# TaiseiNiman/SimpleGaussianSplat_tk71

Measured on AMD Instinct MI355X. Metric: splat-pixel pairs blended per second (grouped cumprod fwd+bwd), higher is better.
Workload: dtype f32; 1 GPU; cfg3: 1920x1080, 1000000 Gaussians, mean 80 splats/pixel (deep heavy-tailed lists); pairs_per_gpu=166335639, pixel_groups_per_gpu=2073600, bytes_per_pair=32, tiles_left_to_the_follow_up_kernel=0, world_size_checked=1, tiles_resolved_through_the_descriptor_tree=1258

## Files before the change

include/grouped_cumprod_hip.h:

```cpp
#ifndef GROUPED_CUMPROD_HIP_H
#define GROUPED_CUMPROD_HIP_H

#include <stddef.h>
#include <stdint.h>

#ifdef __cplusplus
extern "C" {
#endif

#define GCP_OK 0
#define GCP_ERR_INVALID_ARGUMENT 1
#define GCP_ERR_WORKSPACE 2
#define GCP_ERR_HIP 3

#define GCP_ABI_VERSION 4

int gcp_abi_version(void);

const char* gcp_source_hash(void);

int gcp_last_hip_error(void);

const char* gcp_status_string(int status);

size_t gcp_workspace_bytes(int64_t n);

int gcp_workspace_init(void* ws, size_t ws_bytes, void* stream);

int gcp_cumprod_forward(const float* x, const int32_t* key, float* y, int64_t n,
                        void* ws, size_t ws_bytes, void* stream);

int gcp_cumsum_forward(const float* x, const int32_t* key, float* y, int64_t n,
                       void* ws, size_t ws_bytes, void* stream);

int gcp_cumprod_backward(const float* param, const float* param_cumprod,
                         const float* grad_out, const int32_t* inv, float* grad_in,
                         const int32_t* inv_len, int64_t n, int64_t n_groups,
                         void* ws, size_t ws_bytes, void* stream);

int gcp_cumsum_reverse(const float* x, const int32_t* key, float* y, int64_t n,
                       void* ws, size_t ws_bytes, void* stream);

int gcp_cumprod_forward_indexed(const float* x, const int32_t* sorted_key, const int32_t* index, float* y, int64_t n,
                                void* ws, size_t ws_bytes, void* stream);
int gcp_cumsum_forward_indexed(const float* x, const int32_t* sorted_key, const int32_t* index, float* y, int64_t n,
                               void* ws, size_t ws_bytes, void* stream);
int gcp_cumsum_reverse_indexed(const float* x, const int32_t* sorted_key, const int32_t* index, float* y, int64_t n,
                               void* ws, size_t ws_bytes, void* stream);

int gcp_cumprod_forward_carry(const float* x, const int32_t* inv, const float* carry, float* y,
                              int64_t n, int64_t n_groups, void* ws, size_t ws_bytes, void* stream);
int gcp_cumsum_forward_carry(const float* x, const int32_t* inv, const float* carry, float* y,
                             int64_t n, int64_t n_groups, void* ws, size_t ws_bytes, void* stream);
int gcp_cumsum_reverse_carry(const float* x, const int32_t* inv, const float* carry, float* y,
                             int64_t n, int64_t n_groups, void* ws, size_t ws_bytes, void* stream);

int gcp_check_groups(const int32_t* inv, const int32_t* inv_len, int64_t n,
                     int64_t n_groups, int64_t* n_bad, void* stream);

int gcp_check_permutation(const int32_t* index, int64_t n, int64_t* n_bad, void* stream);
int gcp_check_group_ids(const int32_t* inv, int64_t n, int64_t n_groups, int64_t* n_bad, void* stream);
int gcp_set_validate_operands(int on);

int gcp_tile_elems(void);
int gcp_last_fallback_tiles(void* ws, void* stream, int64_t* n_tiles);
int gcp_set_lookback_wait_us(int64_t us);
int gcp_last_lookback_tiles(void* ws, void* stream, int64_t* n_tiles);



int gcp_tile_grid(int32_t width, int32_t height, int32_t* tiles_x, int32_t* tiles_y);

size_t gcp_scan_i32_workspace_bytes(int64_t n);
int gcp_exclusive_scan_i32(const int32_t* in, int32_t* out, int64_t n, void* ws, size_t ws_bytes,
                           void* stream);

int gcp_bin_tiles_count(const int32_t* start_xy, const int32_t* end_xy, int64_t n_gauss,
                        int32_t width, int32_t height, int32_t* tile_off,
                        int64_t* n_tile_pairs_host, void* ws, size_t ws_bytes, void* stream);
size_t gcp_bin_workspace_bytes(int64_t n_gauss, int64_t n_tile_pairs);
int gcp_bin_tiles_fill(const int32_t* start_xy, const int32_t* end_xy, int64_t n_gauss,
                       int32_t width, int32_t height, const int32_t* tile_off,
                       int64_t n_tile_pairs, int32_t* tile_start, int32_t* tile_list, void* ws,
                       size_t ws_bytes, void* stream);

int gcp_bin_tiles(const int32_t* start_xy, const int32_t* end_xy, int64_t n_gauss, int32_t width,
                  int32_t height, int64_t capacity, int32_t* tile_off, int32_t* tile_start,
                  int32_t* tile_list, int32_t* info, void* ws, size_t ws_bytes, void* stream);

size_t gcp_blend_checkpoint_floats(int64_t n_tile_pairs, int32_t width, int32_t height);
int gcp_blend_forward(const int32_t* start_xy, const int32_t* end_xy, const float* mean_xy,
                      const float* vinv, const float* opacity, const float* l_d, int64_t n_gauss,
                      int32_t width, int32_t height, const int32_t* tile_start,
                      const int32_t* tile_list, float* image, float* t_ckpt, void* stream);

size_t gcp_blend_backward_workspace_bytes(int64_t n_tile_pairs);
int gcp_blend_backward(const int32_t* start_xy, const int32_t* end_xy, const float* mean_xy,
                       const float* vinv, const float* opacity, const float* l_d, int64_t n_gauss,
                       int32_t width, int32_t height, const int32_t* tile_off,
                       int64_t n_tile_pairs, const int32_t* tile_start, const int32_t* tile_list,
                       const float* t_ckpt, const float* grad_image, float* grad_mean,
                       float* grad_vinv, float* grad_opacity, float* grad_l, void* ws,
                       size_t ws_bytes, void* stream);

int gcp_blend_forward_depth(const int32_t* start_xy, const int32_t* end_xy, const float* mean_xy,
                            const float* vinv, const float* opacity, const float* l_d, const float* depth,
                            const float* background, int64_t n_gauss, int32_t width, int32_t height,
                            const int32_t* tile_start, const int32_t* tile_list, float* image,
                            float* depth_map, float* alpha_map, float* t_ckpt, void* stream);
size_t gcp_blend_backward_depth_workspace_bytes(int64_t n_tile_pairs, int32_t width, int32_t height);
int gcp_blend_backward_depth(const int32_t* start_xy, const int32_t* end_xy, const float* mean_xy,
                             const float* vinv, const float* opacity, const float* l_d, const float* depth,
                             const float* background, int64_t n_gauss, int32_t width, int32_t height,
                             const int32_t* tile_off, int64_t n_tile_pairs, const int32_t* tile_start,
                             const int32_t* tile_list, const float* t_ckpt, const float* grad_image,
                             const float* grad_depth_map, const float* grad_alpha_map, float* grad_mean,
                             float* grad_vinv, float* grad_opacity, float* grad_l, float* grad_depth,
                             float* grad_background, void* ws, size_t ws_bytes, void* stream);

size_t gcp_sort_workspace_bytes(int64_t n);
int gcp_sort_pairs_u32(const uint32_t* keys_in, int64_t n, int32_t key_bits, uint32_t* keys_out,
// ... 274 lines not shown
```

simplegaussiansplat_tk71_amd/_lib.py:

```python
import ctypes
import os

from . import _build
from ._build import LIB_PATH

_c_void_p = ctypes.c_void_p
_i64 = ctypes.c_int64
_sz = ctypes.c_size_t
_i32 = ctypes.c_int32

SIGNATURES = {
    "gcp_abi_version": (ctypes.c_int, []),
    "gcp_source_hash": (ctypes.c_char_p, []),
    "gcp_last_hip_error": (ctypes.c_int, []),
    "gcp_status_string": (ctypes.c_char_p, [ctypes.c_int]),
    "gcp_workspace_bytes": (_sz, [_i64]),
    "gcp_workspace_init": (ctypes.c_int, [_c_void_p, _sz, _c_void_p]),
    "gcp_cumprod_forward": (ctypes.c_int, [_c_void_p, _c_void_p, _c_void_p, _i64, _c_void_p, _sz, _c_void_p]),
    "gcp_cumsum_forward": (ctypes.c_int, [_c_void_p, _c_void_p, _c_void_p, _i64, _c_void_p, _sz, _c_void_p]),
    "gcp_cumsum_reverse": (ctypes.c_int, [_c_void_p, _c_void_p, _c_void_p, _i64, _c_void_p, _sz, _c_void_p]),
    "gcp_cumprod_forward_indexed": (ctypes.c_int, [_c_void_p] * 4 + [_i64, _c_void_p, _sz, _c_void_p]),
    "gcp_cumsum_forward_indexed": (ctypes.c_int, [_c_void_p] * 4 + [_i64, _c_void_p, _sz, _c_void_p]),
    "gcp_cumsum_reverse_indexed": (ctypes.c_int, [_c_void_p] * 4 + [_i64, _c_void_p, _sz, _c_void_p]),
    "gcp_cumprod_forward_carry": (ctypes.c_int, [_c_void_p] * 4 + [_i64, _i64, _c_void_p, _sz, _c_void_p]),
    "gcp_cumsum_forward_carry": (ctypes.c_int, [_c_void_p] * 4 + [_i64, _i64, _c_void_p, _sz, _c_void_p]),
    "gcp_cumsum_reverse_carry": (ctypes.c_int, [_c_void_p] * 4 + [_i64, _i64, _c_void_p, _sz, _c_void_p]),
    "gcp_cumprod_backward": (
        ctypes.c_int,
        [_c_void_p, _c_void_p, _c_void_p, _c_void_p, _c_void_p, _c_void_p, _i64, _i64, _c_void_p, _sz, _c_void_p],
    ),
    "gcp_check_groups": (ctypes.c_int, [_c_void_p, _c_void_p, _i64, _i64, ctypes.POINTER(_i64), _c_void_p]),
    "gcp_check_permutation": (ctypes.c_int, [_c_void_p, _i64, ctypes.POINTER(_i64), _c_void_p]),
    "gcp_check_group_ids": (ctypes.c_int, [_c_void_p, _i64, _i64, ctypes.POINTER(_i64), _c_void_p]),
    "gcp_set_validate_operands": (ctypes.c_int, [ctypes.c_int]),
    "gcp_tile_elems": (ctypes.c_int, []),
    "gcp_last_fallback_tiles": (ctypes.c_int, [_c_void_p, _c_void_p, ctypes.POINTER(_i64)]),
    "gcp_last_lookback_tiles": (ctypes.c_int, [_c_void_p, _c_void_p, ctypes.POINTER(_i64)]),
    "gcp_set_lookback_wait_us": (ctypes.c_int, [_i64]),
    "gcp_tile_grid": (ctypes.c_int, [_i32, _i32, ctypes.POINTER(_i32), ctypes.POINTER(_i32)]),
    "gcp_scan_i32_workspace_bytes": (_sz, [_i64]),
    "gcp_exclusive_scan_i32": (ctypes.c_int, [_c_void_p, _c_void_p, _i64, _c_void_p, _sz, _c_void_p]),
    "gcp_bin_tiles_count": (
        ctypes.c_int,
        [_c_void_p, _c_void_p, _i64, _i32, _i32, _c_void_p, ctypes.POINTER(_i64), _c_void_p, _sz, _c_void_p],
    ),
    "gcp_bin_workspace_bytes": (_sz, [_i64, _i64]),
    "gcp_bin_tiles_fill": (
        ctypes.c_int,
        [_c_void_p, _c_void_p, _i64, _i32, _i32, _c_void_p, _i64, _c_void_p, _c_void_p, _c_void_p, _sz, _c_void_p],
    ),
    "gcp_bin_tiles": (
        ctypes.c_int,
        [_c_void_p, _c_void_p, _i64, _i32, _i32, _i64, _c_void_p, _c_void_p, _c_void_p, _c_void_p, _c_void_p, _sz, _c_void_p],
    ),
    "gcp_blend_checkpoint_floats": (_sz, [_i64, _i32, _i32]),
    "gcp_blend_forward": (
        ctypes.c_int,
        [_c_void_p] * 6 + [_i64, _i32, _i32, _c_void_p, _c_void_p, _c_void_p, _c_void_p, _c_void_p],
    ),
    "gcp_blend_backward_workspace_bytes": (_sz, [_i64]),
    "gcp_blend_backward": (
        ctypes.c_int,
        [_c_void_p] * 6 + [_i64, _i32, _i32, _c_void_p, _i64] + [_c_void_p] * 8 + [_c_void_p, _sz, _c_void_p],
    ),
    "gcp_blend_forward_depth": (ctypes.c_int, [_c_void_p] * 8 + [_i64, _i32, _i32] + [_c_void_p] * 7),
    "gcp_blend_backward_depth_workspace_bytes": (_sz, [_i64, _i32, _i32]),
    "gcp_blend_backward_depth": (ctypes.c_int, [_c_void_p] * 8 + [_i64, _i32, _i32, _c_void_p, _i64] + [_c_void_p] * 13 + [_sz, _c_void_p]),
    "gcp_gather_f32": (ctypes.c_int, [_c_void_p, _c_void_p, _c_void_p, _i64, _c_void_p]),
    "gcp_unsort_finish": (ctypes.c_int, [_c_void_p] * 5 + [_i64, _i32, _c_void_p]),
    "gcp_sort_workspace_bytes": (_sz, [_i64]),
    "gcp_sort_pairs_u32": (ctypes.c_int, [_c_void_p, _i64, _i32, _c_void_p, _c_void_p, _c_void_p, _sz, _c_void_p]),
    "gcp_sort_rects": (ctypes.c_int, [_c_void_p, _i64, _i32, _i32, _c_void_p, _c_void_p, _c_void_p, _sz, _c_void_p]),
    "gcp_rects_key_range": (ctypes.c_int, [_c_void_p, _i64, _c_void_p, _c_void_p]),
    "gcp_compact_workspace_bytes": (_sz, [_i64]),
    "gcp_compact_finish": (ctypes.c_int, [_c_void_p, _c_void_p, _i64, _i64, _i32, _c_void_p, _c_void_p, _c_void_p, _c_void_p, _c_void_p, _sz, _c_void_p]),
    "gcp_pairs_finish_prepare": (ctypes.c_int, [_c_void_p, _c_void_p, _i64, _c_void_p]),
    "gcp_pairs_finish_boxes": (ctypes.c_int, [_c_void_p, _c_void_p, _i64, _i32, _i32] + [_c_void_p] * 6 + [_i64, _i32, _c_void_p, _i32, _c_void_p]),
    "gcp_compact_kept_workspace_bytes": (_sz, [_i64]),
    "gcp_compact_kept_count": (ctypes.c_int, [_c_void_p, _c_void_p, _i64, _i64, _i64, _c_void_p, _c_void_p, _sz, _c_void_p]),
    "gcp_compact_kept_write": (ctypes.c_int, [_c_void_p, _c_void_p, _i64, _i64, _c_void_p, _c_void_p, _sz, _c_void_p]),
    "gcp_rects_cut_workspace_bytes": (_sz, [_i64, _i64, _i64, _i32, _i64]),
    "gcp_rects_cut": (ctypes.c_int, [_c_void_p, _i32, _i64, _i64, _i64, _i32, _i64] + [_c_void_p] * 6 + [_sz, _c_void_p]),
    "gcp_pixels_range": (ctypes.c_int, [_c_void_p, _i32, _i64, _c_void_p, _c_void_p]),
    "gcp_pixels_min_workspace_bytes": (_sz, [_i32, _i32]),
    "gcp_pixels_min": (ctypes.c_int, [_c_void_p, _i32, _c_void_p, _i64, _i32, _i32, _c_void_p, _c_void_p, _i64, _c_void_p, _c_void_p, _sz, _c_void_p]),
    "gcp_rects_rows_workspace_bytes": (_sz, [_i64]),
    "gcp_rects_rows_capacity": (_i64, [_i64]),
    "gcp_rects_rows": (ctypes.c_int, [_c_void_p, _i64, _i64, _c_void_p, _c_void_p, _c_void_p, _c_void_p, _sz, _c_void_p]),
    "gcp_rects_rows_i64": (ctypes.c_int, [_c_void_p, _i64, _i64, _c_void_p, _c_void_p, _c_void_p, _c_void_p, _sz, _c_void_p]),
    "gcp_rows_rectangles_workspace_bytes": (_sz, [_i64]),
    "gcp_rows_rectangles": (ctypes.c_int, [_c_void_p, _c_void_p, _i64, _c_void_p, _c_void_p, _c_void_p, _sz, _c_void_p]),
    "gcp_rectangle_boxes": (ctypes.c_int, [_c_void_p, _c_void_p, _c_void_p, _i64, _i64, _c_void_p, _c_void_p, _c_void_p, _c_void_p]),
    "gcp_pairs_scan_boxes": (ctypes.c_int, [_c_void_p, _c_void_p, _i64, _i32, _i32] + [_c_void_p] * 5 + [_i64, _i32, _c_void_p, _c_void_p]),
    "gcp_box_sizes": (ctypes.c_int, [_c_void_p, _c_void_p, _i64, _i32, _i32, _c_void_p, _c_void_p]),
    "gcp_expand_rects": (ctypes.c_int, [_c_void_p, _c_void_p, _c_void_p, _i64, _i64, _i32, _i32, _c_void_p, _c_void_p, _c_void_p]),
    "gcp_pixel_lists_count": (ctypes.c_int, [_c_void_p, _c_void_p, _i64, _i32, _i32] + [_c_void_p] * 5),
    "gcp_pixel_lists_fill": (ctypes.c_int, [_c_void_p, _c_void_p, _i64, _i32, _i32] + [_c_void_p] * 8),
    "gcp_project_forward": (ctypes.c_int, [_c_void_p] * 7 + [_i64, _i32, _i32, _i32, _i32, ctypes.c_float] + [_c_void_p] * 5),
    "gcp_project_gather": (ctypes.c_int, [_c_void_p, _c_void_p, _i64] + [_c_void_p] * 11),
    "gcp_adam_step": (ctypes.c_int, [_c_void_p] * 4 + [_i64] + [ctypes.c_double] * 4 + [_i64, _c_void_p]),
    "gcp_adam_step_multi": (ctypes.c_int, [_i32] + [_c_void_p] * 10 + [ctypes.c_double] * 3 + [_c_void_p]),
    "gcp_ssim_blocks": (_i64, [_i64, _i32, _i32]),
    "gcp_ssim_l1_forward": (ctypes.c_int, [_c_void_p, _c_void_p, _i64, _i32, _i32, _c_void_p, ctypes.c_float, ctypes.c_float]
                            + [_c_void_p] * 5),
    "gcp_ssim_l1_backward": (ctypes.c_int, [_c_void_p] * 5 + [_i64, _i32, _i32, _c_void_p, _c_void_p, _c_void_p, _c_void_p]),
    "gcp_image_metrics": (ctypes.c_int, [_c_void_p, _c_void_p, _i64, _i32, _i32, _i32, _c_void_p, ctypes.c_float, ctypes.c_float, _i32]
                          + [_c_void_p] * 3),
    "gcp_exposure_blocks": (_i64, [_i64, _i32, _i32]),
    "gcp_ssim_l1_forward_exposure": (ctypes.c_int, [_c_void_p] * 3 + [_i64, _i32, _i32, _c_void_p, ctypes.c_float, ctypes.c_float]
                                     + [_c_void_p] * 5),
# ... 99 lines not shown
```

simplegaussiansplat_tk71_amd/csrc/gcp_scan.hip:

```cpp

#include <hip/hip_runtime.h>
#include <stdint.h>
#include <stdlib.h>
#include <atomic>
#include <mutex>

#include "gcp_device.hpp"
#include "grouped_cumprod_hip.h"

namespace gcp {
thread_local int t_last_hip_error = 0;
int hip_fail(hipError_t e) {
  t_last_hip_error = (int)e;
  return GCP_ERR_HIP;
}
}

namespace {
using namespace gcp;

typedef float float4_t __attribute__((ext_vector_type(4)));
typedef int int4_t __attribute__((ext_vector_type(4)));

enum : int { M_CUMPROD_FWD = 0, M_CUMSUM_FWD = 1, M_CUMPROD_BWD = 2, M_CUMSUM_REV = 3 };

constexpr int kThreads = 256;
constexpr int kWaves = 4;
constexpr int kRows = 4;
constexpr int kTile = 1024 * kRows;
constexpr int kLbBatch = 5;
constexpr int kLbBatchBwd = 3;
constexpr int kLbChunks = ((kTile / 256 - 1) / kLbBatch) * kLbBatch + 1;
constexpr int kFixBlocks = 256;
constexpr int kFixBlocksQuiet = 32;
constexpr int kWsHeaderBytes = 256;
constexpr int kHdrEpoch = 0;
constexpr int kHdrDone = 1;
constexpr int kHdrUnresolved = 2;
constexpr int kHdrTiles = 3;
constexpr int kHdrDescResolved = 5;
constexpr int kHdrAnyUnresolved = 6;
constexpr int kHdrBarrier = 7;
constexpr unsigned kDOpen = 1u;
constexpr unsigned kDUnresolved = 2u;
constexpr unsigned kDValid = 1u << 15;
constexpr unsigned kDTree = 1u << 16;
constexpr int kLevels = 4;
constexpr int kXcdChunk = 32;
constexpr int kXcdChunkIndexed = 128;
constexpr int kDescWaitUs = 200;

static_assert(kLbChunks * 256 == kTile, "the raw look-back window is exactly the previous tile (the descriptor walk starts at the tile before it)");
static_assert((kLbChunks - 1) % kLbBatch == 0, "chunks after the first are fetched kLbBatch at a time");
static_assert((kLbChunks - 1) % kLbBatchBwd == 0, "chunks after the first are fetched kLbBatchBwd at a time in the backward");

template <int MODE>
struct Mode {
  static constexpr bool kMul = (MODE == M_CUMPROD_FWD);
  static constexpr bool kRev = (MODE == M_CUMPROD_BWD || MODE == M_CUMSUM_REV);
  static constexpr bool kBwd = (MODE == M_CUMPROD_BWD);
  static constexpr int kBatch = kBwd ? kLbBatchBwd : kLbBatch;
};

template <bool MUL>
struct Monoid {
  static __device__ __forceinline__ float identity() { return MUL ? 1.0f : 0.0f; }
  static __device__ __forceinline__ float op(float a, float b) { return MUL ? a * b : a + b; }
};

struct ScanArgs {
  const float* in0;
  const float* in1;
  const float* in2;
  const int* key;
  const int* ends;
  i64 n_groups;
  const float* carry;
  const int* index;
  float* out;
  i64 n;
  i64 ntiles;
  unsigned long long* desc_sets;
  i64 lvl_off[kLevels + 1];
  unsigned* hdr;
  int xcd_remap;
  long long patience;
};

template <bool MUL>
__device__ __forceinline__ float wave_seg_scan(float v, int h, int lane) {
  typedef Monoid<MUL> M;
  const float id = M::identity();
  float t;
  t = dpp_f<0x111, 0xf>(id, v); v = M::op(v, (lane - 1 >= h) ? t : id);
  t = dpp_f<0x112, 0xf>(id, v); v = M::op(v, (lane - 2 >= h) ? t : id);
  t = dpp_f<0x114, 0xf>(id, v); v = M::op(v, (lane - 4 >= h) ? t : id);
  t = dpp_f<0x118, 0xf>(id, v); v = M::op(v, (lane - 8 >= h) ? t : id);
  t = dpp_f<0x142, 0xa>(id, v); v = M::op(v, ((lane & 48) - 1 >= h) ? t : id);
  t = dpp_f<0x143, 0xc>(id, v); v = M::op(v, (31 >= h) ? t : id);
  return v;
}

template <bool MUL>
__device__ __forceinline__ float wave_reduce(float v) {
  typedef Monoid<MUL> M;
  const float id = M::identity();
  v = M::op(v, dpp_f<0x111, 0xf>(id, v));
  v = M::op(v, dpp_f<0x112, 0xf>(id, v));
  v = M::op(v, dpp_f<0x114, 0xf>(id, v));
  v = M::op(v, dpp_f<0x118, 0xf>(id, v));
  v = M::op(v, dpp_f<0x142, 0xa>(id, v));
  v = M::op(v, dpp_f<0x143, 0xc>(id, v));
  return readlane_f(v, 63);
}

template <bool ALIGNED, bool NT = false>
__device__ __forceinline__ float4_t ld4(const float* p) {
  if (ALIGNED) {
    if (NT) return __builtin_nontemporal_load(reinterpret_cast<const float4_t*>(p));
    return *reinterpret_cast<const float4_t*>(p);
  }
  float4_t v; v.x = p[0]; v.y = p[1]; v.z = p[2]; v.w = p[3];
  return v;
}
template <bool ALIGNED, bool NT = false>
__device__ __forceinline__ int4_t ld4(const int* p) {
  if (ALIGNED) {
    if (NT) return __builtin_nontemporal_load(reinterpret_cast<const int4_t*>(p));
    return *reinterpret_cast<const int4_t*>(p);
  }
  int4_t v; v.x = p[0]; v.y = p[1]; v.z = p[2]; v.w = p[3];
  return v;
}
template <bool ALIGNED>
__device__ __forceinline__ void st4(float* p, float4_t v) {
  if (ALIGNED) {
    __builtin_nontemporal_store(v, reinterpret_cast<float4_t*>(p));
    return;
  }
  p[0] = v.x; p[1] = v.y; p[2] = v.z; p[3] = v.w;
}
__device__ __forceinline__ float4_t ld4_guard(const float* base, i64 p0, i64 n, float fill) {
  float4_t v;
  v.x = (p0 + 0 < n) ? base[p0 + 0] : fill;
  v.y = (p0 + 1 < n) ? base[p0 + 1] : fill;
  v.z = (p0 + 2 < n) ? base[p0 + 2] : fill;
  v.w = (p0 + 3 < n) ? base[p0 + 3] : fill;
  return v;
}
__device__ __forceinline__ int4_t ld4_guard(const int* base, i64 p0, i64 n, int fill) {
  int4_t v;
  v.x = (p0 + 0 < n) ? base[p0 + 0] : fill;
  v.y = (p0 + 1 < n) ? base[p0 + 1] : fill;
  v.z = (p0 + 2 < n) ? base[p0 + 2] : fill;
  v.w = (p0 + 3 < n) ? base[p0 + 3] : fill;
  return v;
}
template <bool ALIGNED, bool NT>
__device__ __forceinline__ float4_t ld4_indexed(const float* src, const int* index, i64 p, int4_t& idx) {
  idx = ld4<ALIGNED, NT>(index + p);
  float4_t v; v.x = src[idx.x]; v.y = src[idx.y]; v.z = src[idx.z]; v.w = src[idx.w];
  return v;
}
__device__ __forceinline__ float4_t ld4_indexed_guard(const float* src, const int* index, i64 p0, i64 n, float fill, int4_t& idx) {
  idx = ld4_guard(index, p0, n, 0);
  float4_t v;
  v.x = (p0 + 0 < n) ? src[idx.x] : fill;
  v.y = (p0 + 1 < n) ? src[idx.y] : fill;
  v.z = (p0 + 2 < n) ? src[idx.z] : fill;
  v.w = (p0 + 3 < n) ? src[idx.w] : fill;
  return v;
}
template <bool REV> __device__ __forceinline__ float4_t to_scan_order(float4_t v) {
  if (!REV) return v;
  float4_t r; r.x = v.w; r.y = v.z; r.z = v.y; r.w = v.x;
  return r;
}
template <bool REV> __device__ __forceinline__ int4_t to_scan_order(int4_t v) {
  if (!REV) return v;
  int4_t r; r.x = v.w; r.y = v.z; r.z = v.y; r.w = v.x;
  return r;
}

__device__ __forceinline__ i64 logical_tile(i64 b, i64 ntiles, int xcd_remap) {
  if (!xcd_remap) return b;
  const int lg = xcd_remap - 1 + 3;
  const i64 full = (ntiles >> lg) << lg;
  if (b >= full) return b;
  const i64 g = b >> lg, r = b & (((i64)1 << lg) - 1);
  return (g << lg) + ((r & 7) << (lg - 3)) + (r >> 3);
}

__device__ __forceinline__ unsigned long long pack_desc(float agg, unsigned flags, int first_head) {
  return ((unsigned long long)(flags | kDValid | ((unsigned)first_head << 2)) << 32) | __builtin_bit_cast(unsigned, agg);
}

constexpr int kEndIters = 4;
constexpr int kBitWords = 256 * kRows / 32;

__device__ __forceinline__ void wave_sync_lds() {
  __builtin_amdgcn_fence(__ATOMIC_RELEASE, "wavefront");
  __builtin_amdgcn_wave_barrier();
  __builtin_amdgcn_fence(__ATOMIC_ACQUIRE, "wavefront");
}

__device__ __forceinline__ bool group_ends(const ScanArgs& a, unsigned* bits, i64 wlo, i64 whi, int ga, int gb, int lane,
                                          i64& gend) {
  if (lane < kBitWords) bits[lane] = 0u;
  wave_sync_lds();
  if (!(wlo <= whi && ga >= 0 && ga <= gb && (i64)gb < a.n_groups && (i64)gb - ga + 2 <= 64 * kEndIters)) return false;
  const int last = gb - ga + 1;
  int e[kEndIters];
#pragma unroll
  for (int it = 0; it < kEndIters; ++it) {
    const int j = it * 64 + lane;
    e[it] = 0;
    if (j <= last && ga - 1 + j >= 0) e[it] = a.ends[ga - 1 + j];
  }
  bool bad = false;
  gend = 0;
#pragma unroll
  for (int it = 0; it < kEndIters; ++it) {
    const int j = it * 64 + lane;
    const int prev = dpp_i<0x138, 0xf>(it ? __builtin_amdgcn_readlane(e[it > 0 ? it - 1 : 0], 63) : 0, e[it]);
    const i64 ej = e[it];
    if (j >= 1 && j <= last) {
      bad = bad || e[it] <= prev;
      const i64 p = ej - 1;
      if (p >= wlo && p <= whi) atomicOr(bits + ((p - wlo) >> 5), 1u << ((p - wlo) & 31));
    }
    if (j == 0) bad = bad || ej > wlo;
    if (j == 1) bad = bad || ej <= wlo;
    if (j == last - 1) bad = bad || ej > whi;
    if (j == last) bad = bad || ej <= whi;
    if ((last >> 6) == it) gend = (i64)__builtin_amdgcn_readlane(e[it], last & 63);
  }
  wave_sync_lds();
  return __ballot(bad) == 0ull;
}

template <int MODE, bool ALIGNED, bool FULL, bool CARRY, bool FIXUP = false, bool INDEXED = false, bool INPLACE = false>
__device__ __forceinline__ void scan_tile(const ScanArgs& a, const i64 lt, float* s_wv, int* s_wf,
                                          float* s_tc, int* s_fh, unsigned* s_bits, const float fix_carry = 0.0f) {
  typedef Mode<MODE> MD;
  constexpr bool REV = MD::kRev;
  constexpr bool BWD = MD::kBwd;
  typedef Monoid<MD::kMul> M;
  const float id = M::identity();
  constexpr int WT = 256 * kRows;

  const int lane = threadIdx.x & 63;
  const int w = threadIdx.x >> 6;
  const i64 n = a.n;
  const i64 pt = REV ? (a.ntiles - 1 - lt) : lt;
  const i64 base = pt * (i64)kTile;
  unsigned long long* const desc = a.desc_sets + (a.hdr[kHdrEpoch] & 1u);

  const int wu = __builtin_amdgcn_readfirstlane(w);
  i64 wlo = 0, whi = -1;
  int ga = 0, gb = -1;
  if constexpr (BWD) {
    wlo = base + kTile - (i64)(wu + 1) * WT;
    whi = base + kTile - 1 - (i64)wu * WT;
    if (whi > n - 1) whi = n - 1;
  }

  const bool nt_main = w < kWaves - 1;
  float4_t v[kRows];
  int4_t kk[kRows];
  float4_t xp[BWD ? kRows : 1];
  int4_t ix[INDEXED ? kRows : 1];
  static_assert(!(INDEXED && BWD), "the backward has no indexed form");
  int4_t lb_ix;
  i64 p0[kRows];
  auto load_keys = [&](int r) {
    if (FULL) {
      if (nt_main) kk[r] = ld4<ALIGNED, true>(a.key + p0[r]);
      else kk[r] = ld4<ALIGNED>(a.key + p0[r]);
    } else {
      kk[r] = ld4_guard(a.key, p0[r], n, 0);
    }
    kk[r] = to_scan_order<REV>(kk[r]);
  };
#pragma unroll
  for (int r = 0; r < kRows; ++r) {
    const int q = w * WT + r * 256 + lane * 4;
    p0[r] = REV ? (base + kTile - 4 - q) : (base + q);
    if constexpr (!BWD) load_keys(r);
    if (FULL) {
      if (nt_main) {
        if constexpr (BWD) {
          v[r] = ld4<ALIGNED, true>(a.in2 + p0[r]) * ld4<ALIGNED, true>(a.in1 + p0[r]);
        } else if constexpr (INDEXED) {
          v[r] = ld4_indexed<ALIGNED, true>(a.in0, a.index, p0[r], ix[r]);
        } else {
          v[r] = ld4<ALIGNED, true>(a.in0 + p0[r]);
        }
      } else {
        if constexpr (BWD) {
          v[r] = ld4<ALIGNED>(a.in2 + p0[r]) * ld4<ALIGNED>(a.in1 + p0[r]);
        } else if constexpr (INDEXED) {
          v[r] = ld4_indexed<ALIGNED, false>(a.in0, a.index, p0[r], ix[r]);
        } else {
          v[r] = ld4<ALIGNED>(a.in0 + p0[r]);
        }
      }
      if constexpr (BWD) xp[r] = ld4<ALIGNED, true>(a.in0 + p0[r]);
    } else {
      if constexpr (BWD) {
        const float4_t g = ld4_guard(a.in2, p0[r], n, 0.0f);
        const float4_t c = ld4_guard(a.in1, p0[r], n, 0.0f);
        xp[r] = ld4_guard(a.in0, p0[r], n, 1.0f);
        v[r] = g * c;
      } else if constexpr (INDEXED) {
        v[r] = ld4_indexed_guard(a.in0, a.index, p0[r], n, id, ix[r]);
      } else {
        v[r] = ld4_guard(a.in0, p0[r], n, id);
      }
    }
    v[r] = to_scan_order<REV>(v[r]);
    if constexpr (BWD) xp[r] = to_scan_order<REV>(xp[r]);
  }

  if constexpr (BWD) {
    if (wlo <= whi) { ga = a.key[wlo]; gb = a.key[whi]; }
  }

  const i64 pn = REV ? (base + kTile - (i64)w * WT) : (base + (i64)w * WT - 1);
  const bool nb_exists = (pn >= 0) && (pn < n);
  int nbk = 0;
  if (!BWD && nb_exists) nbk = a.key[pn];

  const bool do_lb = !FIXUP && !INPLACE && (w == 0) && (lt > 0);
  float4_t lbv = {id, id, id, id};
  float4_t lbc = {id, id, id, id};
  int4_t lbk = {0, 0, 0, 0};
  i64 lbp = 0;
  if (do_lb) {
    lbp = REV ? (base + kTile + lane * 4) : (base - (lane * 4 + 4));
    if (!REV) {
      lbk = ld4<ALIGNED>(a.key + lbp);
      if constexpr (BWD) lbv = ld4<ALIGNED>(a.in2 + lbp) * ld4<ALIGNED>(a.in1 + lbp);
      else if constexpr (INDEXED) lbv = ld4_indexed<ALIGNED, false>(a.in0, a.index, lbp, lb_ix);
      else lbv = ld4<ALIGNED>(a.in0 + lbp);
    } else if (BWD && base + kTile + 256 <= n) {
      lbv = ld4<ALIGNED>(a.in2 + lbp);
      lbc = ld4<ALIGNED>(a.in1 + lbp);
    } else {
      if constexpr (!BWD) lbk = ld4_guard(a.key, lbp, n, 0);
      if constexpr (BWD) { lbv = ld4_guard(a.in2, lbp, n, 0.0f); lbc = ld4_guard(a.in1, lbp, n, 0.0f); }
      else if constexpr (INDEXED) lbv = ld4_indexed_guard(a.in0, a.index, lbp, n, id, lb_ix);
      else lbv = ld4_guard(a.in0, lbp, n, id);
    }
  }

  bool from_ends = false;
  i64 gend = 0;
  unsigned* const wbits = s_bits + kBitWords * wu;
  if constexpr (BWD) {
    from_ends = group_ends(a, wbits, wlo, whi, ga, gb, lane, gend);
    if (!from_ends) {
#pragma unroll
      for (int r = 0; r < kRows; ++r) load_keys(r);
      if (nb_exists) nbk = a.key[pn];
      if (do_lb) lbk = ld4_guard(a.key, lbp, n, 0);
    }
  }

  float s[kRows][4];
  float eloc[kRows];
  float rowtot[kRows];
  unsigned long long hmask[kRows];
  unsigned openbits = 0;
  unsigned lanes_open = 0;

#pragma unroll
  for (int r = 0; r < kRows; ++r) {
    int lane0_prev;
    if (r == 0) lane0_prev = nbk;
    else lane0_prev = __builtin_amdgcn_readlane(kk[r - 1].w, 63);
    const int pk = dpp_i<0x138, 0xf>(lane0_prev, kk[r].w);

    bool f0, f1, f2, f3;
    if (BWD && from_ends) {
      const int off = WT - 4 - r * 256 - lane * 4;
      const unsigned nib = (wbits[off >> 5] >> (off & 31)) & 0xfu;
      f0 = (nib >> 3) & 1u; f1 = (nib >> 2) & 1u; f2 = (nib >> 1) & 1u; f3 = nib & 1u;
      if (FULL) {
        f0 = f0 || ((lt == 0) && (w == 0) && (r == 0) && (lane == 0));
      } else {
        const i64 p = p0[r];
        f0 = (p + 3 < n) && (f0 || p + 3 == n - 1);
        f1 = (p + 2 < n) && (f1 || p + 2 == n - 1);
        f2 = (p + 1 < n) && (f2 || p + 1 == n - 1);
        f3 = (p + 0 < n) && (f3 || p + 0 == n - 1);
      }
    } else if (FULL) {
      const bool first_of_array = (lt == 0) && (w == 0) && (r == 0) && (lane == 0);
      f0 = first_of_array || (kk[r].x != pk);
      f1 = kk[r].y != kk[r].x;
      f2 = kk[r].z != kk[r].y;
      f3 = kk[r].w != kk[r].z;
    } else {
      bool val[4], pex[4];
#pragma unroll
      for (int k = 0; k < 4; ++k) {
        const i64 p = REV ? (p0[r] + 3 - k) : (p0[r] + k);
        val[k] = p < n;
        pex[k] = REV ? (p + 1 < n) : (p > 0);
      }
      f0 = val[0] && (!pex[0] || kk[r].x != pk);
      f1 = val[1] && (!pex[1] || kk[r].y != kk[r].x);
      f2 = val[2] && (!pex[2] || kk[r].z != kk[r].y);
      f3 = val[3] && (!pex[3] || kk[r].w != kk[r].z);
    }
    if constexpr (CARRY) {
      if (f0) v[r].x = M::op(a.carry[kk[r].x], v[r].x);
      if (f1) v[r].y = M::op(a.carry[kk[r].y], v[r].y);
      if (f2) v[r].z = M::op(a.carry[kk[r].z], v[r].z);
      if (f3) v[r].w = M::op(a.carry[kk[r].w], v[r].w);
    }
    const float s0 = v[r].x;
    const float s1 = f1 ? v[r].y : M::op(s0, v[r].y);
    const float s2 = f2 ? v[r].z : M::op(s1, v[r].z);
    const float s3 = f3 ? v[r].w : M::op(s2, v[r].w);
    s[r][0] = s0; s[r][1] = s1; s[r][2] = s2; s[r][3] = s3;
    const bool m0 = !f0, m1 = m0 && !f1, m2 = m1 && !f2, m3 = m2 && !f3;
    openbits |= ((unsigned)m0 | ((unsigned)m1 << 1) | ((unsigned)m2 << 2) | ((unsigned)m3 << 3)) << (4 * r);

    const unsigned long long mask = __ballot(!m3);
    hmask[r] = mask;
    const unsigned long long upto = mask & (~0ull >> (63 - lane));
    const int h = upto ? (63 - __clzll(upto)) : -1;
    if ((mask & ((1ull << lane) - 1ull)) == 0ull) lanes_open |= 1u << r;

    const float inc = wave_seg_scan<MD::kMul>(s3, h, lane);
    eloc[r] = dpp_f<0x138, 0xf>(id, inc);
    rowtot[r] = readlane_f(inc, 63);
  }

  float wagg = id;
  bool whead = false;
#pragma unroll
  for (int r = 0; r < kRows; ++r) {
    wagg = hmask[r] ? rowtot[r] : M::op(wagg, rowtot[r]);
    whead = whead || (hmask[r] != 0ull);
  }
  int wfh = WT;
#pragma unroll
  for (int r = kRows - 1; r >= 0; --r) {
    if (hmask[r]) {
      const int hl = __builtin_ctzll(hmask[r]);
      const unsigned ob = (unsigned)__builtin_amdgcn_readlane((int)openbits, hl);
      wfh = r * 256 + hl * 4 + __builtin_popcount((ob >> (4 * r)) & 0xfu);
    }
  }
  if (lane == 0) { s_wv[w] = wagg; s_wf[w] = whead ? 1 : 0; s_fh[w] = wfh; }

  if (w == 0) {
    float tc = FIXUP ? fix_carry : id;
    int unresolved = 0;
    if (do_lb) {
      const int k0 = from_ends ? 0 : __builtin_amdgcn_readfirstlane(kk[0].x);
      auto process = [&](float4_t cv, int4_t ck, i64 cp, int j) -> bool {
        const float4_t lv = REV ? cv : to_scan_order<true>(cv);
        const int4_t lk = REV ? ck : to_scan_order<true>(ck);
        bool c0, c1, c2, c3;
// ... 677 lines not shown
  GCP_HIP(hipMemsetAsync(ws, 0, ws_bytes, (hipStream_t)stream));
  return GCP_OK;
}

int gcp_cumprod_forward(const float* x, const int32_t* key, float* y, int64_t n, void* ws,
                        size_t ws_bytes, void* stream) {
  return launch_scan<M_CUMPROD_FWD>(x, nullptr, nullptr, key, y, n, ws, ws_bytes, stream);
}

int gcp_cumsum_forward(const float* x, const int32_t* key, float* y, int64_t n, void* ws,
                       size_t ws_bytes, void* stream) {
  return launch_scan<M_CUMSUM_FWD>(x, nullptr, nullptr, key, y, n, ws, ws_bytes, stream);
}

int gcp_cumsum_reverse(const float* x, const int32_t* key, float* y, int64_t n, void* ws,
                       size_t ws_bytes, void* stream) {
  return launch_scan<M_CUMSUM_REV>(x, nullptr, nullptr, key, y, n, ws, ws_bytes, stream);
}

int gcp_cumprod_forward_indexed(const float* x, const int32_t* sorted_key, const int32_t* index, float* y, int64_t n,
                                void* ws, size_t ws_bytes, void* stream) {
  if (n > 0 && !index) return GCP_ERR_INVALID_ARGUMENT;
  if (validate_operands()) {
    const int st = check_permutation_impl(index, n, nullptr, (hipStream_t)stream);
    if (st != GCP_OK) return st;
  }
  return launch_scan<M_CUMPROD_FWD>(x, nullptr, nullptr, sorted_key, y, n, ws, ws_bytes, stream, nullptr, index);
}

int gcp_cumsum_forward_indexed(const float* x, const int32_t* sorted_key, const int32_t* index, float* y, int64_t n,
                               void* ws, size_t ws_bytes, void* stream) {
  if (n > 0 && !index) return GCP_ERR_INVALID_ARGUMENT;
  if (validate_operands()) {
    const int st = check_permutation_impl(index, n, nullptr, (hipStream_t)stream);
    if (st != GCP_OK) return st;
  }
  return launch_scan<M_CUMSUM_FWD>(x, nullptr, nullptr, sorted_key, y, n, ws, ws_bytes, stream, nullptr, index);
}

int gcp_cumsum_reverse_indexed(const float* x, const int32_t* sorted_key, const int32_t* index, float* y, int64_t n,
                               void* ws, size_t ws_bytes, void* stream) {
  if (n > 0 && !index) return GCP_ERR_INVALID_ARGUMENT;
  if (validate_operands()) {
    const int st = check_permutation_impl(index, n, nullptr, (hipStream_t)stream);
    if (st != GCP_OK) return st;
  }
  return launch_scan<M_CUMSUM_REV>(x, nullptr, nullptr, sorted_key, y, n, ws, ws_bytes, stream, nullptr, index);
}

int gcp_cumprod_forward_carry(const float* x, const int32_t* inv, const float* carry, float* y, int64_t n,
                              int64_t n_groups, void* ws, size_t ws_bytes, void* stream) {
  if (n > 0 && (!carry || n_groups <= 0)) return GCP_ERR_INVALID_ARGUMENT;
  if (validate_operands()) {
    const int st = check_group_ids_impl(inv, n, n_groups, nullptr, (hipStream_t)stream);
    if (st != GCP_OK) return st;
  }
  return launch_scan<M_CUMPROD_FWD>(x, nullptr, nullptr, inv, y, n, ws, ws_bytes, stream, carry);
}

int gcp_cumsum_forward_carry(const float* x, const int32_t* inv, const float* carry, float* y, int64_t n,
                             int64_t n_groups, void* ws, size_t ws_bytes, void* stream) {
  if (n > 0 && (!carry || n_groups <= 0)) return GCP_ERR_INVALID_ARGUMENT;
  if (validate_operands()) {
    const int st = check_group_ids_impl(inv, n, n_groups, nullptr, (hipStream_t)stream);
    if (st != GCP_OK) return st;
  }
  return launch_scan<M_CUMSUM_FWD>(x, nullptr, nullptr, inv, y, n, ws, ws_bytes, stream, carry);
}

int gcp_cumsum_reverse_carry(const float* x, const int32_t* inv, const float* carry, float* y, int64_t n,
                             int64_t n_groups, void* ws, size_t ws_bytes, void* stream) {
  if (n > 0 && (!carry || n_groups <= 0)) return GCP_ERR_INVALID_ARGUMENT;
  if (validate_operands()) {
    const int st = check_group_ids_impl(inv, n, n_groups, nullptr, (hipStream_t)stream);
    if (st != GCP_OK) return st;
  }
  return launch_scan<M_CUMSUM_REV>(x, nullptr, nullptr, inv, y, n, ws, ws_bytes, stream, carry);
}

int gcp_cumprod_backward(const float* param, const float* param_cumprod, const float* grad_out,
                         const int32_t* inv, float* grad_in, const int32_t* inv_len, int64_t n,
                         int64_t n_groups, void* ws, size_t ws_bytes, void* stream) {
  if (n > 0 && (!inv_len || n_groups <= 0)) return GCP_ERR_INVALID_ARGUMENT;
  return launch_scan<M_CUMPROD_BWD>(param, param_cumprod, grad_out, inv, grad_in, n, ws, ws_bytes,
                                    stream, nullptr, nullptr, inv_len, n_groups);
}

int gcp_check_groups(const int32_t* inv, const int32_t* inv_len, int64_t n, int64_t n_groups,
                     int64_t* n_bad, void* stream_) {
  hipStream_t stream = (hipStream_t)stream_;
  if (!n_bad || n < 0) return GCP_ERR_INVALID_ARGUMENT;
  *n_bad = 0;
  if (n == 0) return GCP_OK;
  if (!inv || !inv_len || n_groups <= 0) return GCP_ERR_INVALID_ARGUMENT;
  unsigned long long* d = nullptr;
  GCP_HIP(hipMalloc((void**)&d, sizeof(unsigned long long)));
  hipError_t e = hipMemsetAsync(d, 0, sizeof(unsigned long long), stream);
  if (e == hipSuccess) {
    i64 blocks = (n + 255) / 256;
    if (blocks > 4096) blocks = 4096;
    hipLaunchKernelGGL(gcp_check_groups_kernel, dim3((unsigned)blocks), dim3(256), 0, stream, inv,
                       inv_len, (i64)n, (i64)n_groups, d);
    e = hipGetLastError();
  }
  unsigned long long h = 0;
  if (e == hipSuccess) e = hipMemcpyAsync(&h, d, sizeof(h), hipMemcpyDeviceToHost, stream);
  if (e == hipSuccess) e = hipStreamSynchronize(stream);
  (void)hipFree(d);
  if (e != hipSuccess) return hip_fail(e);
  *n_bad = (int64_t)h;
  return GCP_OK;
}

int gcp_check_permutation(const int32_t* index, int64_t n, int64_t* n_bad, void* stream) {
  return check_permutation_impl(index, (i64)n, n_bad, (hipStream_t)stream);
}

int gcp_check_group_ids(const int32_t* inv, int64_t n, int64_t n_groups, int64_t* n_bad, void* stream) {
  return check_group_ids_impl(inv, (i64)n, (i64)n_groups, n_bad, (hipStream_t)stream);
}

int gcp_set_validate_operands(int on) {
  g_validate.store(on ? 1 : 0, std::memory_order_relaxed);
  return GCP_OK;
}

int gcp_tile_elems(void) { return kTile; }

int gcp_set_lookback_wait_us(int64_t us) {
  g_patience_us.store(us < 0 ? -1 : (long long)us, std::memory_order_relaxed);
  return GCP_OK;
}

int gcp_last_fallback_tiles(void* ws, void* stream_, int64_t* n_tiles) {
  hipStream_t stream = (hipStream_t)stream_;
  if (!n_tiles) return GCP_ERR_INVALID_ARGUMENT;
  *n_tiles = 0;
  if (!ws) {
    int dev = 0;
    GCP_HIP(hipGetDevice(&dev));
    std::lock_guard<std::mutex> lock(g_ws_mutex);
    if (dev < 0 || dev >= 64 || !g_ws[dev].ptr) return GCP_OK;
    ws = g_ws[dev].ptr;
  }
  unsigned h = 0;
  GCP_HIP(hipMemcpyAsync(&h, (const char*)ws + 4 * kHdrUnresolved, sizeof(h), hipMemcpyDeviceToHost, stream));
  GCP_HIP(hipStreamSynchronize(stream));
  *n_tiles = (int64_t)h;
  return GCP_OK;
}

int gcp_last_lookback_tiles(void* ws, void* stream_, int64_t* n_tiles) {
  hipStream_t stream = (hipStream_t)stream_;
  if (!n_tiles) return GCP_ERR_INVALID_ARGUMENT;
  *n_tiles = 0;
  if (!ws) {
    int dev = 0;
    GCP_HIP(hipGetDevice(&dev));
    std::lock_guard<std::mutex> lock(g_ws_mutex);
    if (dev < 0 || dev >= 64 || !g_ws[dev].ptr) return GCP_OK;
    ws = g_ws[dev].ptr;
  }
  unsigned h = 0;
  GCP_HIP(hipMemcpyAsync(&h, (const char*)ws + 4 * kHdrDescResolved, sizeof(h), hipMemcpyDeviceToHost, stream));
  GCP_HIP(hipStreamSynchronize(stream));
  *n_tiles = (int64_t)h;
// ... 5 lines not shown
```

simplegaussiansplat_tk71_amd/grouped_cumprod.py:

```python
import ctypes

import torch

from . import _lib

__all__ = [
    "grouped_cumprod_forward",
    "grouped_cumsum_forward",
    "grouped_cumprod_backward",
    "grouped_cumsum_reverse",
    "grouped_cumprod_forward_indexed",
    "grouped_cumsum_forward_indexed",
    "grouped_cumsum_reverse_indexed",
    "grouped_cumprod_forward_carry",
    "grouped_cumsum_forward_carry",
    "grouped_cumsum_reverse_carry",
    "Workspace",
    "check_groups",
    "check_permutation",
    "check_group_ids",
    "set_validate_operands",
    "last_fallback_tiles",
    "last_lookback_tiles",
    "set_lookback_wait_us",
# ... 83 lines not shown
    if status:
        _lib.check(status, fn_name)


def _forward(fn_name, x, key, y, workspace=None):
    _require(isinstance(key, torch.Tensor), "pixel_index: expected a torch.Tensor")
    n = key.numel()
    dev = key.device
    _check_tensor(key, "pixel_index", torch.int32, dev)
    _check_tensor(x, "unti_opacity", torch.float32, dev, n)
    _check_tensor(y, "out", torch.float32, dev, n)
    if n == 0:
        return
    inplace = y.data_ptr() == x.data_ptr()
    _no_alias(y, "out", *(() if inplace else ((x, "unti_opacity"),)), (key, "pixel_index"))
    _launch(fn_name, dev, n, (x.data_ptr(), key.data_ptr(), y.data_ptr()), workspace=workspace)


def grouped_cumprod_forward(unti_opacity, pixel_index, out, *, workspace=None):
    _forward("gcp_cumprod_forward", unti_opacity, pixel_index, out, workspace)


def grouped_cumsum_forward(unti_opacity, pixel_index, out, *, workspace=None):
    _forward("gcp_cumsum_forward", unti_opacity, pixel_index, out, workspace)


def grouped_cumsum_reverse(x, key, out, *, workspace=None):
    _forward("gcp_cumsum_reverse", x, key, out, workspace)


def _forward_indexed(fn_name, x, sorted_key, index, y):
    _require(isinstance(sorted_key, torch.Tensor), "sorted_key: expected a torch.Tensor")
    n = sorted_key.numel()
    dev = sorted_key.device
    _check_tensor(sorted_key, "sorted_key", torch.int32, dev)
    _check_tensor(index, "index", torch.int32, dev, n)
    _check_tensor(x, "x", torch.float32, dev, n)
    _check_tensor(y, "out", torch.float32, dev, n)
    if n == 0:
        return
    _no_alias(y, "out", (x, "x"), (sorted_key, "sorted_key"), (index, "index"))
    _launch(fn_name, dev, n, (x.data_ptr(), sorted_key.data_ptr(), index.data_ptr(), y.data_ptr()))


def grouped_cumprod_forward_indexed(x, sorted_key, index, out):
    _forward_indexed("gcp_cumprod_forward_indexed", x, sorted_key, index, out)


def grouped_cumsum_forward_indexed(x, sorted_key, index, out):
    _forward_indexed("gcp_cumsum_forward_indexed", x, sorted_key, index, out)


def grouped_cumsum_reverse_indexed(x, sorted_key, index, out):
    _forward_indexed("gcp_cumsum_reverse_indexed", x, sorted_key, index, out)


def _forward_carry(fn_name, x, inv, carry, y):
    _require(isinstance(inv, torch.Tensor), "inv: expected a torch.Tensor")
    n = inv.numel()
    dev = inv.device
    _check_tensor(inv, "inv", torch.int32, dev)
    _check_tensor(x, "x", torch.float32, dev, n)
    _check_tensor(y, "out", torch.float32, dev, n)
    _check_tensor(carry, "carry", torch.float32, dev)
    if n == 0:
        return
    _require(carry.numel() > 0, "carry: empty for a non-empty input")
    _no_alias(y, "out", (x, "x"), (inv, "inv"), (carry, "carry"))
    _launch(fn_name, dev, n, (x.data_ptr(), inv.data_ptr(), carry.data_ptr(), y.data_ptr()), (carry.numel(),))


def grouped_cumprod_forward_carry(x, inv, carry, out):
    _forward_carry("gcp_cumprod_forward_carry", x, inv, carry, out)


def grouped_cumsum_forward_carry(x, inv, carry, out):
    _forward_carry("gcp_cumsum_forward_carry", x, inv, carry, out)


def grouped_cumsum_reverse_carry(x, inv, carry, out):
    _forward_carry("gcp_cumsum_reverse_carry", x, inv, carry, out)


def grouped_cumprod_backward(param, param_cumprod, grad_out, inv, grad_in, inv_len, *, workspace=None):
    _require(isinstance(param, torch.Tensor), "param: expected a torch.Tensor")
    n = param.numel()
    dev = param.device
    _check_tensor(param, "param", torch.float32, dev)
    _check_tensor(param_cumprod, "param_cumprod", torch.float32, dev, n)
    _check_tensor(grad_out, "grad_out", torch.float32, dev, n)
    _check_tensor(inv, "inv", torch.int32, dev, n)
    _check_tensor(grad_in, "grad_in", torch.float32, dev, n)
    _check_tensor(inv_len, "inv_len", torch.int32, dev)
    if n == 0:
        return
    _require(inv_len.numel() > 0, "inv_len: empty for a non-empty input")
    _no_alias(grad_in, "grad_in", (param, "param"), (param_cumprod, "param_cumprod"), (grad_out, "grad_out"), (inv, "inv"),
              (inv_len, "inv_len"))
    _launch(
        "gcp_cumprod_backward",
        dev,
        n,
        (param.data_ptr(), param_cumprod.data_ptr(), grad_out.data_ptr(), inv.data_ptr(), grad_in.data_ptr(),
         inv_len.data_ptr()),
        (inv_len.numel(),),
        workspace=workspace,
    )


def check_groups(inv, inv_len):
    dev = inv.device
    n = inv.numel()
    _check_tensor(inv, "inv", torch.int32, dev)
    _check_tensor(inv_len, "inv_len", torch.int32, dev)
    lib = _lib.load()
    bad = ctypes.c_int64(0)
    with torch.cuda.device(dev):
        stream = torch.cuda.current_stream(dev).cuda_stream
        status = lib.gcp_check_groups(inv.data_ptr(), inv_len.data_ptr(), n, inv_len.numel(), ctypes.byref(bad), stream)
    _lib.check(status, "gcp_check_groups")
    return bad.value


def check_permutation(index):
    dev = index.device
    _check_tensor(index, "index", torch.int32, dev)
    bad = ctypes.c_int64(0)
    with torch.cuda.device(dev):
        status = _lib.load().gcp_check_permutation(index.data_ptr(), index.numel(), ctypes.byref(bad),
                                                   torch.cuda.current_stream(dev).cuda_stream)
    if status not in (0, 1):
        _lib.check(status, "gcp_check_permutation")
    return bad.value


def check_group_ids(inv, n_groups):
    dev = inv.device
    _check_tensor(inv, "inv", torch.int32, dev)
    _require(int(n_groups) > 0 or inv.numel() == 0, "n_groups: must be positive for a non-empty input")
    bad = ctypes.c_int64(0)
    with torch.cuda.device(dev):
        status = _lib.load().gcp_check_group_ids(inv.data_ptr(), inv.numel(), int(n_groups), ctypes.byref(bad),
                                                 torch.cuda.current_stream(dev).cuda_stream)
    if status not in (0, 1):
        _lib.check(status, "gcp_check_group_ids")
    return bad.value


def set_validate_operands(on):
    _lib.check(_lib.load().gcp_set_validate_operands(1 if on else 0), "gcp_set_validate_operands")


def _last_stat(fn_name, device):
    device = torch.device("cuda", torch.cuda.current_device()) if device is None else torch.device(device)
    lib = _lib.load()
    out = ctypes.c_int64(0)
    with torch.cuda.device(device):
        stream = torch.cuda.current_stream(device).cuda_stream
        hit = _workspaces.get((device.index, stream))
        if hit is None:
            return 0
        status = getattr(lib, fn_name)(hit.tensor.data_ptr(), stream, ctypes.byref(out))
    _lib.check(status, fn_name)
    return out.value


def last_fallback_tiles(device=None):
    return _last_stat("gcp_last_fallback_tiles", device)


def last_lookback_tiles(device=None):
    return _last_stat("gcp_last_lookback_tiles", device)


def set_lookback_wait_us(us):
    _lib.check(_lib.load().gcp_set_lookback_wait_us(int(us)), "gcp_set_lookback_wait_us")


def tile_elems():
    return _lib.load().gcp_tile_elems()
```

Before: 217.0 billion pairs/s.

## Recompute forward cumprod in backward scan instead of loading param_cumprod

The default cumprod backward now rebuilds the forward prefix products inside each wave from param, using a segmented downward multiply-scan anchored on one cumprod value per wave. It stops streaming the full param_cumprod array and keeps the old load-based path as a separately named 'given' entry point. This removes one 4-byte load per element from a bandwidth-bound kernel. In exchange it adds extra wave-level scan work, ballots and DPP shuffles, and its rounding can differ from the stored forward values.

New measurement: 235.6 billion pairs/s (median of 6 runs). +8.6%, better.

```diff
diff --git a/include/grouped_cumprod_hip.h b/include/grouped_cumprod_hip.h
--- a/include/grouped_cumprod_hip.h
+++ b/include/grouped_cumprod_hip.h
@@ -37,6 +37,11 @@
                          const float* grad_out, const int32_t* inv, float* grad_in,
                          const int32_t* inv_len, int64_t n, int64_t n_groups,
                          void* ws, size_t ws_bytes, void* stream);
+
+int gcp_cumprod_backward_given(const float* param, const float* param_cumprod,
+                               const float* grad_out, const int32_t* inv, float* grad_in,
+                               const int32_t* inv_len, int64_t n, int64_t n_groups,
+                               void* ws, size_t ws_bytes, void* stream);
 
 int gcp_cumsum_reverse(const float* x, const int32_t* key, float* y, int64_t n,
                        void* ws, size_t ws_bytes, void* stream);
diff --git a/simplegaussiansplat_tk71_amd/_lib.py b/simplegaussiansplat_tk71_amd/_lib.py
--- a/simplegaussiansplat_tk71_amd/_lib.py
+++ b/simplegaussiansplat_tk71_amd/_lib.py
@@ -26,6 +26,10 @@
     "gcp_cumsum_forward_carry": (ctypes.c_int, [_c_void_p] * 4 + [_i64, _i64, _c_void_p, _sz, _c_void_p]),
     "gcp_cumsum_reverse_carry": (ctypes.c_int, [_c_void_p] * 4 + [_i64, _i64, _c_void_p, _sz, _c_void_p]),
     "gcp_cumprod_backward": (
+        ctypes.c_int,
+        [_c_void_p, _c_void_p, _c_void_p, _c_void_p, _c_void_p, _c_void_p, _i64, _i64, _c_void_p, _sz, _c_void_p],
+    ),
+    "gcp_cumprod_backward_given": (
         ctypes.c_int,
         [_c_void_p, _c_void_p, _c_void_p, _c_void_p, _c_void_p, _c_void_p, _i64, _i64, _c_void_p, _sz, _c_void_p],
     ),
diff --git a/simplegaussiansplat_tk71_amd/csrc/gcp_scan.hip b/simplegaussiansplat_tk71_amd/csrc/gcp_scan.hip
--- a/simplegaussiansplat_tk71_amd/csrc/gcp_scan.hip
+++ b/simplegaussiansplat_tk71_amd/csrc/gcp_scan.hip
@@ -22,7 +22,7 @@
 typedef float float4_t __attribute__((ext_vector_type(4)));
 typedef int int4_t __attribute__((ext_vector_type(4)));
 
-enum : int { M_CUMPROD_FWD = 0, M_CUMSUM_FWD = 1, M_CUMPROD_BWD = 2, M_CUMSUM_REV = 3 };
+enum : int { M_CUMPROD_FWD = 0, M_CUMSUM_FWD = 1, M_CUMPROD_BWD = 2, M_CUMSUM_REV = 3, M_CUMPROD_BWD_RECOMPUTE = 4 };
 
 constexpr int kThreads = 256;
 constexpr int kWaves = 4;
@@ -57,8 +57,9 @@
 template <int MODE>
 struct Mode {
   static constexpr bool kMul = (MODE == M_CUMPROD_FWD);
-  static constexpr bool kRev = (MODE == M_CUMPROD_BWD || MODE == M_CUMSUM_REV);
-  static constexpr bool kBwd = (MODE == M_CUMPROD_BWD);
+  static constexpr bool kRev = (MODE == M_CUMPROD_BWD || MODE == M_CUMSUM_REV || MODE == M_CUMPROD_BWD_RECOMPUTE);
+  static constexpr bool kBwd = (MODE == M_CUMPROD_BWD || MODE == M_CUMPROD_BWD_RECOMPUTE);
+  static constexpr bool kRecompute = (MODE == M_CUMPROD_BWD_RECOMPUTE);
   static constexpr int kBatch = kBwd ? kLbBatchBwd : kLbBatch;
 };
 
@@ -101,6 +102,20 @@
   return v;
 }
 
+__device__ __forceinline__ float wave_seg_scan_down_mul(float v, int hp, int lane) {
+  float t;
+  t = dpp_f<0x101, 0xf>(1.0f, v); v = v * ((lane + 1 <= hp) ? t : 1.0f);
+  t = dpp_f<0x102, 0xf>(1.0f, v); v = v * ((lane + 2 <= hp) ? t : 1.0f);
+  t = dpp_f<0x104, 0xf>(1.0f, v); v = v * ((lane + 4 <= hp) ? t : 1.0f);
+  t = dpp_f<0x108, 0xf>(1.0f, v); v = v * ((lane + 8 <= hp) ? t : 1.0f);
+#pragma unroll
+  for (int q = 2; q >= 0; --q) {
+    const float c = readlane_f(v, 16 * (q + 1));
+    v = v * (((lane >> 4) == q && hp >= 16 * (q + 1)) ? c : 1.0f);
+  }
+  return v;
+}
+
 template <bool MUL>
 __device__ __forceinline__ float wave_reduce(float v) {
   typedef Monoid<MUL> M;
@@ -205,7 +220,7 @@
 }
 
 __device__ __forceinline__ bool group_ends(const ScanArgs& a, unsigned* bits, i64 wlo, i64 whi, int ga, int gb, int lane,
-                                          i64& gend) {
+                                          i64& gend, i64& gstart) {
   if (lane < kBitWords) bits[lane] = 0u;
   wave_sync_lds();
   if (!(wlo <= whi && ga >= 0 && ga <= gb && (i64)gb < a.n_groups && (i64)gb - ga + 2 <= 64 * kEndIters)) return false;
@@ -219,6 +234,7 @@
   }
   bool bad = false;
   gend = 0;
+  gstart = (i64)__builtin_amdgcn_readlane(e[0], 0);
 #pragma unroll
   for (int it = 0; it < kEndIters; ++it) {
     const int j = it * 64 + lane;
@@ -245,6 +261,7 @@
   typedef Mode<MODE> MD;
   constexpr bool REV = MD::kRev;
   constexpr bool BWD = MD::kBwd;
+  constexpr bool RECOMP = MD::kRecompute;
   typedef Monoid<MD::kMul> M;
   const float id = M::identity();
   constexpr int WT = 256 * kRows;
@@ -289,7 +306,9 @@
     if constexpr (!BWD) load_keys(r);
     if (FULL) {
       if (nt_main) {
-        if constexpr (BWD) {
+        if constexpr (RECOMP) {
+          v[r] = ld4<ALIGNED, true>(a.in2 + p0[r]);
+        } else if constexpr (BWD) {
           v[r] = ld4<ALIGNED, true>(a.in2 + p0[r]) * ld4<ALIGNED, true>(a.in1 + p0[r]);
         } else if constexpr (INDEXED) {
           v[r] = ld4_indexed<ALIGNED, true>(a.in0, a.index, p0[r], ix[r]);
@@ -297,7 +316,9 @@
           v[r] = ld4<ALIGNED, true>(a.in0 + p0[r]);
         }
       } else {
-        if constexpr (BWD) {
+        if constexpr (RECOMP) {
+          v[r] = ld4<ALIGNED>(a.in2 + p0[r]);
+        } else if constexpr (BWD) {
           v[r] = ld4<ALIGNED>(a.in2 + p0[r]) * ld4<ALIGNED>(a.in1 + p0[r]);
         } else if constexpr (INDEXED) {
           v[r] = ld4_indexed<ALIGNED, false>(a.in0, a.index, p0[r], ix[r]);
@@ -307,7 +328,10 @@
       }
       if constexpr (BWD) xp[r] = ld4<ALIGNED, true>(a.in0 + p0[r]);
     } else {
-      if constexpr (BWD) {
+      if constexpr (RECOMP) {
+        v[r] = ld4_guard(a.in2, p0[r], n, 0.0f);
+        xp[r] = ld4_guard(a.in0, p0[r], n, 1.0f);
+      } else if constexpr (BWD) {
         const float4_t g = ld4_guard(a.in2, p0[r], n, 0.0f);
         const float4_t c = ld4_guard(a.in1, p0[r], n, 0.0f);
         xp[r] = ld4_guard(a.in0, p0[r], n, 1.0f);
@@ -324,6 +348,10 @@
 
   if constexpr (BWD) {
     if (wlo <= whi) { ga = a.key[wlo]; gb = a.key[whi]; }
+  }
+  float anchor = 1.0f;
+  if constexpr (RECOMP) {
+    if (wlo > 0 && wlo <= whi) anchor = a.in1[wlo - 1];
   }
 
   const i64 pn = REV ? (base + kTile - (i64)w * WT) : (base + (i64)w * WT - 1);
@@ -357,13 +385,18 @@
   bool from_ends = false;
   i64 gend = 0;
   unsigned* const wbits = s_bits + kBitWords * wu;
+  i64 gstart = 0;
+  int kbelow = 0;
   if constexpr (BWD) {
-    from_ends = group_ends(a, wbits, wlo, whi, ga, gb, lane, gend);
+    from_ends = group_ends(a, wbits, wlo, whi, ga, gb, lane, gend, gstart);
     if (!from_ends) {
 #pragma unroll
       for (int r = 0; r < kRows; ++r) load_keys(r);
       if (nb_exists) nbk = a.key[pn];
       if (do_lb) lbk = ld4_guard(a.key, lbp, n, 0);
+      if constexpr (RECOMP) {
+        if (wlo > 0 && wlo <= whi) kbelow = a.key[wlo - 1];
+      }
     }
   }
 
@@ -374,6 +407,57 @@
   unsigned openbits = 0;
   unsigned lanes_open = 0;
 
+  unsigned ebits = 0;
+  if constexpr (RECOMP) {
+    unsigned long long e3[kRows];
+#pragma unroll
+    for (int r = 0; r < kRows; ++r) {
+      unsigned nib;
+      if (from_ends) {
+        const int off = WT - 4 - r * 256 - lane * 4;
+        nib = (wbits[off >> 5] >> (off & 31)) & 0xfu;
+      } else {
+        const int up = (r == 0) ? nbk : __builtin_amdgcn_readlane(kk[r > 0 ? r - 1 : 0].w, 63);
+        const int pk = dpp_i<0x138, 0xf>(up, kk[r].w);
+        nib = (unsigned)(kk[r].w != kk[r].z) | ((unsigned)(kk[r].z != kk[r].y) << 1) | ((unsigned)(kk[r].y != kk[r].x) << 2) |
+              ((unsigned)(kk[r].x != pk) << 3);
+      }
+      if (FULL) {
+        if ((lt == 0) && (w == 0) && (r == 0) && (lane == 0)) nib |= 8u;
+      } else {
+        const i64 m = n - p0[r];
+        nib = (m >= 4) ? (m == 4 ? (nib | 8u) : nib) : (m <= 0 ? 0u : ((nib | (1u << (m - 1))) & ((1u << m) - 1u)));
+      }
+      ebits |= nib << (4 * r);
+      e3[r] = __ballot((nib & 8u) != 0u);
+    }
+    const bool low_head = (wlo == 0) || (from_ends ? (gstart == wlo) : (kbelow != ga));
+    float C = anchor;
+#pragma unroll
+    for (int r = kRows - 1; r >= 0; --r) {
+      const bool below = (r == kRows - 1) ? low_head : ((e3[r < kRows - 1 ? r + 1 : r] & 1ull) != 0ull);
+      const bool F0 = (lane == 63) ? below : (((e3[r] >> 1) >> lane) & 1ull) != 0ull;
+      const bool F1 = (ebits >> (4 * r)) & 1u, F2 = (ebits >> (4 * r + 1)) & 1u, F3 = (ebits >> (4 * r + 2)) & 1u;
+      const float q0 = xp[r].w;
+      const float q1 = F1 ? xp[r].z : q0 * xp[r].z;
+      const float q2 = F2 ? xp[r].y : q1 * xp[r].y;
+      const float q3 = F3 ? xp[r].x : q2 * xp[r].x;
+      const bool n0 = !F0, n1 = n0 && !F1, n2 = n1 && !F2, n3 = n2 && !F3;
+      const unsigned long long pm = __ballot(!n3);
+      const unsigned long long from = pm >> lane;
+      const int hp = from ? lane + __builtin_ctzll(from) : 64;
+      const float inc = wave_seg_scan_down_mul(q3, hp, lane);
+      const float ex = dpp_f<0x130, 0xf>(1.0f, inc);
+      const float e = (((pm >> 1) >> lane) == 0ull) ? C * ex : ex;
+      v[r].w *= n0 ? e * q0 : q0;
+      v[r].z *= n1 ? e * q1 : q1;
+      v[r].y *= n2 ? e * q2 : q2;
+      v[r].x *= n3 ? e * q3 : q3;
+      const float tot = readlane_f(inc, 0);
+      C = pm ? tot : C * tot;
+    }
+  }
+
 #pragma unroll
   for (int r = 0; r < kRows; ++r) {
     int lane0_prev;
@@ -382,7 +466,9 @@
     const int pk = dpp_i<0x138, 0xf>(lane0_prev, kk[r].w);
 
     bool f0, f1, f2, f3;
-    if (BWD && from_ends) {
+    if constexpr (RECOMP) {
+      f0 = (ebits >> (4 * r + 3)) & 1u; f1 = (ebits >> (4 * r + 2)) & 1u; f2 = (ebits >> (4 * r + 1)) & 1u; f3 = (ebits >> (4 * r)) & 1u;
+    } else if (BWD && from_ends) {
       const int off = WT - 4 - r * 256 - lane * 4;
       const unsigned nib = (wbits[off >> 5] >> (off & 31)) & 0xfu;
       f0 = (nib >> 3) & 1u; f1 = (nib >> 2) & 1u; f2 = (nib >> 1) & 1u; f3 = nib & 1u;
@@ -1226,6 +1312,14 @@
                          const int32_t* inv, float* grad_in, const int32_t* inv_len, int64_t n,
                          int64_t n_groups, void* ws, size_t ws_bytes, void* stream) {
   if (n > 0 && (!inv_len || n_groups <= 0)) return GCP_ERR_INVALID_ARGUMENT;
+  return launch_scan<M_CUMPROD_BWD_RECOMPUTE>(param, param_cumprod, grad_out, inv, grad_in, n, ws, ws_bytes,
+                                              stream, nullptr, nullptr, inv_len, n_groups);
+}
+
+int gcp_cumprod_backward_given(const float* param, const float* param_cumprod, const float* grad_out,
+                               const int32_t* inv, float* grad_in, const int32_t* inv_len, int64_t n,
+                               int64_t n_groups, void* ws, size_t ws_bytes, void* stream) {
+  if (n > 0 && (!inv_len || n_groups <= 0)) return GCP_ERR_INVALID_ARGUMENT;
   return launch_scan<M_CUMPROD_BWD>(param, param_cumprod, grad_out, inv, grad_in, n, ws, ws_bytes,
                                     stream, nullptr, nullptr, inv_len, n_groups);
 }
diff --git a/simplegaussiansplat_tk71_amd/grouped_cumprod.py b/simplegaussiansplat_tk71_amd/grouped_cumprod.py
--- a/simplegaussiansplat_tk71_amd/grouped_cumprod.py
+++ b/simplegaussiansplat_tk71_amd/grouped_cumprod.py
@@ -189,7 +189,7 @@
     _forward_carry("gcp_cumsum_reverse_carry", x, inv, carry, out)
 
 
-def grouped_cumprod_backward(param, param_cumprod, grad_out, inv, grad_in, inv_len, *, workspace=None):
+def grouped_cumprod_backward(param, param_cumprod, grad_out, inv, grad_in, inv_len, *, workspace=None, given=False):
     _require(isinstance(param, torch.Tensor), "param: expected a torch.Tensor")
     n = param.numel()
     dev = param.device
@@ -205,7 +205,7 @@
     _no_alias(grad_in, "grad_in", (param, "param"), (param_cumprod, "param_cumprod"), (grad_out, "grad_out"), (inv, "inv"),
               (inv_len, "inv_len"))
     _launch(
-        "gcp_cumprod_backward",
+        "gcp_cumprod_backward_given" if given else "gcp_cumprod_backward",
         dev,
         n,
         (param.data_ptr(), param_cumprod.data_ptr(), grad_out.data_ptr(), inv.data_ptr(), grad_in.data_ptr(),
```
